# ToniChopp/ECAMP

Measured on AMD Instinct MI355X. Metric: pretrain image-report pairs/sec (ViT-B/16, 224^2, seq=128), higher is better.
Workload: dtype bf16

## Files before the change

### ecamp_amd/csrc/gemm.hip

```cpp
#include "common.h"
#include <stdlib.h>
#include <string.h>
#include <stdint.h>

#include "gemm_args.h"
void attn_set_head_mode(int on);
#include "gemm_q8.h"
#include "gemm_q16.h"

#define BM 128
#define BN 128
#define BK 64

__device__ __forceinline__ int swz(int row) { return (row >> 1) & 7; }

__device__ __forceinline__ void g2r_kc(const bf16_t* P, long ld, int row0, int nrows, int k0, int kend, int tid,
                                       uint4 (&r)[4]) {
#pragma unroll
    for (int i = 0; i < 4; ++i) {
        int c = tid + 256 * i;
        int row = c >> 3, kc = c & 7;
        int gr = row0 + row, gk = k0 + kc * 8;
        r[i] = (gr < nrows && gk < kend) ? *reinterpret_cast<const uint4*>(P + (long)gr * ld + gk) : make_uint4(0, 0, 0, 0);
    }
// ... 562 lines not shown
        }
    }
    hipLaunchKernelGGL(gemm_fp8_kernel, dim3(g.nbm * g.nbn), dim3(256), 0, stream, g, scale_a, scale_b);
    if (prof) ecamp_prof_end(stream);
    if (q8_out) {
        const long n4 = M * N / 4;
        int nb = (int)((n4 + 255) / 256);
        if (nb > 4096) nb = 4096;
        hipLaunchKernelGGL(quant_fp8_delayed_kernel<bf16_t>, dim3(nb), dim3(256), 0, stream, (const bf16_t*)C, q8_scale, (unsigned int*)q8_out, q8_amax_slots, n4);
    }
    ECAMP_LAUNCH_CHECK();
    return 0;
}

static int p8_num_cu() {
    static int ncu = 0;
    if (!ncu) {
        int dev = 0;
        (void)hipGetDevice(&dev);
        if (hipDeviceGetAttribute(&ncu, hipDeviceAttributeMultiprocessorCount, dev) != hipSuccess || ncu <= 0) ncu = 256;
        const char* cap = getenv("ECAMP_GEMM_GRID_CAP");
        if (cap && atoi(cap) >= 32 && atoi(cap) < ncu) {
            ncu = atoi(cap);
            fprintf(stderr, "[ecamp_hip] WARNING: ECAMP_GEMM_GRID_CAP=%d -- a development switch: every persistent GEMM of this process runs on %d "
                            "workgroups instead of one per CU\n", ncu, ncu);
        }
    }
    return ncu;
}
static int g_p8_wgrad = 1;
static int g_p8_wgrad_reserve = 0;
static int g_q8_bwd_grid = 0;

static int g_q8_mode = -2;
static int q8_env() {
    static const int v = getenv("ECAMP_GEMM_Q8") ? atoi(getenv("ECAMP_GEMM_Q8")) : -1;
    return g_q8_mode != -2 ? g_q8_mode : v;
}
static int q8_epi(const float* bias, const void* residual, const void* pre_out, const void* gmul, int act, int out_f32) {
    if (out_f32) return (!bias && !residual && !pre_out && !gmul && !act) ? 4 : -1;
    if (gmul) return (!bias && !pre_out && (act == 0 || act == 2)) ? 3 : -1;
    if (pre_out || act) return (pre_out && (act == 1 || act == 2) && !residual) ? 1 : -1;
    if (residual) return 2;
    return 0;
}
static long g_q8_launches = 0;
extern "C" int64_t ecamp_gemm_q8_launches(void) { return g_q8_launches; }
typedef void (*q8_fn)(GemmArgs);
static int g_q8_sch = -1;
static int q8_sch() {
    static const int v = getenv("ECAMP_Q8_SCH") ? atoi(getenv("ECAMP_Q8_SCH")) : 7;
    return g_q8_sch >= 0 ? g_q8_sch : v;
}
static q8_fn q8_pick(int a_kc, int b_kc, int epi, bool rowsum) {
    const int sch = q8_sch();
#define Q8S(A, B, E, R) ((q8_fn)gemm_bf16_q8_kernel<A, B, E, 0, R, 1>)
    if (a_kc && b_kc && (sch & 1)) return epi == 0 ? Q8S(true, true, 0, false) : epi == 1 ? Q8S(true, true, 1, false) : epi == 2 ? Q8S(true, true, 2, false) : (q8_fn) nullptr;
    if (a_kc && !b_kc && (sch & 2)) return epi == 0 ? Q8S(true, false, 0, false) : epi == 2 ? Q8S(true, false, 2, false) : epi == 3 ? Q8S(true, false, 3, false) : (q8_fn) nullptr;
    if (!a_kc && !b_kc && epi == 4 && (sch & 4)) return rowsum ? Q8S(false, false, 4, true) : Q8S(false, false, 4, false);
#undef Q8S
    if (a_kc && b_kc) return epi == 0 ? gemm_bf16_q8_kernel<true, true, 0> : epi == 1 ? gemm_bf16_q8_kernel<true, true, 1> : epi == 2 ? gemm_bf16_q8_kernel<true, true, 2> : (q8_fn) nullptr;
    if (a_kc && !b_kc) return epi == 0 ? gemm_bf16_q8_kernel<true, false, 0> : epi == 2 ? gemm_bf16_q8_kernel<true, false, 2> : epi == 3 ? gemm_bf16_q8_kernel<true, false, 3> : (q8_fn) nullptr;
    if (!a_kc && !b_kc && epi == 4) return rowsum ? gemm_bf16_q8_kernel<false, false, 4, 0, true> : gemm_bf16_q8_kernel<false, false, 4, 0, false>;
    return nullptr;
}
static bool q8_legal(const void* A, const void* B, const void* C, int64_t M, int64_t N, int64_t K, int a_kc, int64_t lda, int b_kc, int64_t ldb, int64_t ldc,
                     const float* bias, const void* residual, int64_t ldr, const void* pre_out, int64_t ldp, const void* gmul, int64_t ldg, int act,
                     int dtype, int out_f32, int split_k, const float* splitk_ws, const float* rowsum) {
    if (dtype != ECAMP_BF16) return false;
    const int epi = q8_epi(bias, residual, pre_out, gmul, act, out_f32);
    if (epi < 0 || !q8_pick(a_kc, b_kc, epi, rowsum != nullptr)) return false;
    if (split_k < 1) split_k = 1;
    if (split_k > 1 && epi != 4) return false;
    long kps = (K + split_k - 1) / split_k;
    kps = (kps + 63) / 64 * 64;
    const long ns = (K + kps - 1) / kps, last = K - (ns - 1) * kps;
    if (kps < 128 || last <= 64) return false;
    auto al16 = [](const void* q) { return (reinterpret_cast<uintptr_t>(q) & 15) == 0; };
    const long lim = 0x7fffffffl;
    if (N % 8 || lda % 8 || ldb % 8 || !al16(A) || !al16(B) || !al16(C)) return false;
    if ((a_kc ? M * lda : K * lda) * 2 > lim || (b_kc ? N * ldb : K * ldb) * 2 > lim) return false;
    if (!a_kc && M % 8) return false;
    if (split_k > 1) { if (!al16(splitk_ws) || (long)split_k * M * N * 4 > lim) return false; }
    else if (ldc % 8 || M * ldc * (epi == 4 ? 4 : 2) > lim) return false;
    if (bias && !al16(bias)) return false;
    if (pre_out && (ldp % 8 || !al16(pre_out) || M * ldp * 2 > lim)) return false;
    if (gmul && (ldg % 8 || !al16(gmul) || M * ldg * 2 > lim)) return false;
    if (residual && (ldr % 8 || !al16(residual) || M * ldr * 2 > lim)) return false;
    return true;
}

static int g_q16_mode = -1;
static int q16_mode() {
    static const int v = getenv("ECAMP_Q16") ? atoi(getenv("ECAMP_Q16")) : 1;
    return g_q16_mode >= 0 ? g_q16_mode : v;
}
static long g_q16_launches = 0;
extern "C" int64_t ecamp_gemm_q16_launches(void) { return g_q16_launches; }
static double q16_cost(int64_t M, int64_t N, int tn, int ncu) {
    const long tiles = (long)ceil_div(M, 256) * ceil_div(N, tn);
    return (double)((tiles + ncu - 1) / ncu) * (tn == 192 ? 0.79 : 1.0);
}
typedef void (*q16_fn)(GemmArgs);
static q16_fn q16_pick(int b_kc, int epi, int nw) {
    if (b_kc) {
        if (nw == 8) return epi == 0 ? (q16_fn)gemm_bf16_q16_kernel<0, 8, true> : (q16_fn)gemm_bf16_q16_kernel<2, 8, true>;
        return epi == 0 ? (q16_fn)gemm_bf16_q16_kernel<0, 6, true> : (q16_fn)gemm_bf16_q16_kernel<2, 6, true>;
    }
    if (nw == 8) return epi == 0 ? (q16_fn)gemm_bf16_q16_kernel<0, 8, false> : (q16_fn)gemm_bf16_q16_kernel<2, 8, false>;
    return epi == 0 ? (q16_fn)gemm_bf16_q16_kernel<0, 6, false> : (q16_fn)gemm_bf16_q16_kernel<2, 6, false>;
}

extern "C" int ecamp_set_option(const char* name, int32_t value) {
    ECAMP_CHECK_ARG(name != nullptr, "set_option: null name");
    if (strcmp(name, "q16_mode") == 0) { g_q16_mode = (value >= 0 && value <= 3) ? value : -1; return 0; }
    if (strcmp(name, "q8_mode") == 0) { g_q8_mode = (value == 0 || value == 2) ? value : -1; return 0; }
    if (strcmp(name, "p8_wgrad") == 0) { g_p8_wgrad = value ? 1 : 0; return 0; }
    if (strcmp(name, "p8_wgrad_reserve_cus") == 0) { g_p8_wgrad_reserve = value < 0 ? 0 : value; return 0; }
    if (strcmp(name, "q8_bwd_grid") == 0) { g_q8_bwd_grid = value < 0 ? 0 : value; return 0; }
    if (strcmp(name, "q8_sch") == 0) { g_q8_sch = value; return 0; }
    if (strcmp(name, "attn_head") == 0) { attn_set_head_mode(value); return 0; }
    return ecamp_set_error(-1, "set_option: unknown option '%s'", name);
}

static long q8_min_items() {
    static const long v = getenv("ECAMP_Q8_MIN_ITEMS") ? atol(getenv("ECAMP_Q8_MIN_ITEMS")) : (long)(0.5 * p8_num_cu());
    return v;
}
static long wgrad_target_items(int ncu) {
    static const long v = getenv("ECAMP_WGRAD_ITEMS") ? atol(getenv("ECAMP_WGRAD_ITEMS")) : 0;
    return v > 0 ? v : ncu;
}

extern "C" int ecamp_gemm_suggest_split(int64_t M, int64_t N, int64_t K, int a_kc, int b_kc, int dtype) {
    if (M <= 0 || N <= 0 || K <= 0) return 1;
    int ncu = p8_num_cu();
    if (!(a_kc && b_kc) && g_p8_wgrad_reserve > 0 && ncu - g_p8_wgrad_reserve >= 64) ncu -= g_p8_wgrad_reserve;
    const long tiles = (long)ceil_div(M, 128) * ceil_div(N, 128);
    long s_old = 1024 / tiles;
    if (s_old < 1) s_old = 1;
    const long cap = (K + 255) / 256;
    if (s_old > cap) s_old = cap;
    if (dtype != ECAMP_BF16 || q8_env() == 0 || (a_kc != 0) != (b_kc != 0) || (!a_kc && !b_kc && !g_p8_wgrad)) return (int)s_old;
    const long t8 = (long)ceil_div(M, 256) * ceil_div(N, 256);
    const long tgt = (!a_kc && !b_kc) ? wgrad_target_items(ncu) : ncu;
    int best = 1;
    double best_score = -1.0;
    for (int sp = 1; sp <= 32; ++sp) {
        if (sp > 1 && K / sp < 512) break;
        const long items = t8 * sp;
        const long rounds = (items + tgt - 1) / tgt;
        const double score = (double)items / (double)(rounds * tgt) - 0.012 * (sp - 1);
        if (score > best_score + 1e-9) { best_score = score; best = sp; }
    }
    return t8 * best >= q8_min_items() ? best : (int)s_old;
}

extern "C" int64_t ecamp_gemm_workspace_bytes(int64_t M, int64_t N, int64_t K, int32_t split_k) {
    (void)K;
    return split_k > 1 && M > 0 && N > 0 ? (int64_t)split_k * M * N * 4 : 0;
}

extern "C" int ecamp_gemm(const void* A, const void* B, void* C, int64_t M, int64_t N, int64_t K, int a_kc, int64_t lda,
                          int b_kc, int64_t ldb, int64_t ldc, const float* bias, const void* residual, int64_t ldr,
                          void* pre_out, int64_t ldp, const void* gmul, int64_t ldg, int act, float alpha, const float* alpha_dev, int dtype,
                          int out_f32, int accumulate, int split_k, float* splitk_ws, float* rowsum, hipStream_t stream) {
    ECAMP_CHECK_ARG(A && B && C, "ecamp_gemm: null operand");
    ECAMP_CHECK_ARG(M > 0 && N > 0 && K > 0, "ecamp_gemm: bad shape %ld %ld %ld", (long)M, (long)N, (long)K);
    ECAMP_CHECK_ARG(dtype == ECAMP_F32 || dtype == ECAMP_BF16, "ecamp_gemm: bad dtype %d", dtype);
    ECAMP_CHECK_ARG(act >= 0 && act <= 2, "ecamp_gemm: act=%d (0 none, 1 GELU, 2 GELU with the saved derivative)", act);
    ECAMP_CHECK_ARG(act != 2 || (dtype == ECAMP_BF16 && !out_f32 && ((pre_out != nullptr) != (gmul != nullptr))),
                    "ecamp_gemm: act=2 (saved derivative) is the bf16 forward form with pre_out or the data-gradient form with gmul");
    const int vec = dtype == ECAMP_BF16 ? 8 : 4;
// ... 390 lines not shown
```

### ecamp_amd/csrc/gemm_q8.h

```cpp
#pragma once
#include "gemm_args.h"
#include <type_traits>

typedef __attribute__((ext_vector_type(16))) float f32x16;
typedef hw_h16x8 hw_bf16x8;
typedef __attribute__((ext_vector_type(4))) short q8_v4s16;
typedef unsigned int q8_u32x4_t __attribute__((ext_vector_type(4)));

#define Q8_HALF 16384
#define Q8_GLDS16(SRC, DST) \
    __builtin_amdgcn_global_load_lds((const void __attribute__((address_space(1)))*)(SRC), (void __attribute__((address_space(3)))*)(DST), 16, 0, 0)

static __device__ __attribute__((aligned(16))) unsigned int q8_zero16[4] = {0u, 0u, 0u, 0u};

struct Q8Item {
    int m0, n0, kbeg, kend, nt, z, ncol;
};
template <int KT_SHIFT = 6>
__device__ __forceinline__ Q8Item q8_decode(const GemmArgs& g, int v, int total) {
    const unsigned f = (unsigned)xcd_remap(v, total), ntile = (unsigned)(g.nbm * g.nbn);
    const unsigned z = f / ntile, tile = f - z * ntile;
    const unsigned gw = 8u * (unsigned)g.nbn, grp = tile / gw, in = tile - grp * gw, first = grp * 8u;
    const unsigned gsz = min(8u, (unsigned)g.nbm - first);
    const unsigned nb = in / gsz, mb = first + (in - nb * gsz);
// ... 327 lines not shown
        } else {                                                                                                         \
            acc[tm_][nh_] = ECAMP_MFMA_32x32x16(FN[nh_].get(), FM[tm_].get(), (ZERO) ? zero16 : acc[tm_][nh_]); \
        }                                                                                                                \
    } while (0)

    const int esz = EPI == 4 ? 4 : 2;
    const long ldo = (EPI == 4 && g.partial) ? (long)g.N : g.ldc;
    const __amdgpu_buffer_rsrc_t rC = __builtin_amdgcn_make_buffer_rsrc(
        (EPI == 4 && g.partial) ? (void*)g.partial : g.C, 0,
        (int)(unsigned)(((EPI == 4 && g.partial) ? (long)g.nsplit * g.M : (long)g.M) * ldo * esz), 0x00020000);
    const __amdgpu_buffer_rsrc_t rP = __builtin_amdgcn_make_buffer_rsrc(EPI == 1 ? g.pre_out : g.C, 0, (int)(unsigned)((long)g.M * g.ldp * 2), 0x00020000);
    const __amdgpu_buffer_rsrc_t rQ = __builtin_amdgcn_make_buffer_rsrc((F8 && EPI == 1 && g.q8_out) ? g.q8_out : g.C, 0, (int)(unsigned)((long)g.M * g.ldc), 0x00020000);
    float q8_max = 0.f;
    const unsigned lane_o = (unsigned)((l31 * ldo + 8 * lh) * esz);
    const unsigned lane_p = (unsigned)((l31 * g.ldp + 8 * lh) * 2);
    const unsigned lane_g = (unsigned)((l31 * g.ldg + 8 * lh) * 2);
    const unsigned lane_r = (unsigned)((l31 * g.ldr + 8 * lh) * 2);
    const __amdgpu_buffer_rsrc_t rG = __builtin_amdgcn_make_buffer_rsrc((void*)(EPI == 3 ? g.gmul : g.C), 0, (int)(unsigned)((long)g.M * g.ldg * 2), 0x00020000);
    const __amdgpu_buffer_rsrc_t rR = __builtin_amdgcn_make_buffer_rsrc((void*)((EPI == 2 || EPI == 3) && g.residual ? g.residual : g.C), 0,
                                                                        (int)(unsigned)((long)g.M * g.ldr * 2), 0x00020000);
    q8_u32x4 bq[2][2][2];
    typedef unsigned q8_u32x4s __attribute__((ext_vector_type(4)));
    constexpr bool HAS_BIAS = (EPI <= 2) && !ITEMS;
    const unsigned bias_lane = (unsigned)((wc * 64 + 8 * lh) * 4);
    auto bias_request = [&](int tn0) __attribute__((always_inline)) {
        if constexpr (HAS_BIAS) {
            if (g.bias) {
                const unsigned long long bp = (unsigned long long)g.bias;
                const q8_u32x4s rs_ = {(unsigned)bp, (unsigned)(bp >> 32) & 0xffffu, (unsigned)g.N * 4u, 0x00020000u};
                const unsigned vo = (unsigned)tn0 * 4u + bias_lane;
#define Q8_BOF(NH_, GQ_, H_) "n"(((NH_) * 32 + (GQ_) * 16 + (H_) * 4) * 4)
                asm volatile("s_nop 4\n\t"
                             "buffer_load_dwordx4 %0, %8, %9, 0 offen offset:%10\n\t"
                             "buffer_load_dwordx4 %1, %8, %9, 0 offen offset:%11\n\t"
                             "buffer_load_dwordx4 %2, %8, %9, 0 offen offset:%12\n\t"
                             "buffer_load_dwordx4 %3, %8, %9, 0 offen offset:%13\n\t"
                             "buffer_load_dwordx4 %4, %8, %9, 0 offen offset:%14\n\t"
                             "buffer_load_dwordx4 %5, %8, %9, 0 offen offset:%15\n\t"
                             "buffer_load_dwordx4 %6, %8, %9, 0 offen offset:%16\n\t"
                             "buffer_load_dwordx4 %7, %8, %9, 0 offen offset:%17"
                             : "=&v"(bq[0][0][0]), "=&v"(bq[0][0][1]), "=&v"(bq[0][1][0]), "=&v"(bq[0][1][1]),
                               "=&v"(bq[1][0][0]), "=&v"(bq[1][0][1]), "=&v"(bq[1][1][0]), "=&v"(bq[1][1][1])
                             : "v"(vo), "s"(rs_), Q8_BOF(0, 0, 0), Q8_BOF(0, 0, 1), Q8_BOF(0, 1, 0), Q8_BOF(0, 1, 1),
                               Q8_BOF(1, 0, 0), Q8_BOF(1, 0, 1), Q8_BOF(1, 1, 0), Q8_BOF(1, 1, 1));
#undef Q8_BOF
            }
        }
    };
    auto bias_landed = [&]() __attribute__((always_inline)) {
        if constexpr (HAS_BIAS)
            asm volatile("" : "+v"(bq[0][0][0]), "+v"(bq[0][0][1]), "+v"(bq[0][1][0]), "+v"(bq[0][1][1]),
                              "+v"(bq[1][0][0]), "+v"(bq[1][0][1]), "+v"(bq[1][1][0]), "+v"(bq[1][1][1]));
    };
    auto store_quadrant = [&](int tm0, int tn0, int tz, auto mh_c, auto nh_c) {
        constexpr int MH = decltype(mh_c)::value, NH = decltype(nh_c)::value;
        constexpr int NTM = 2;
        if (DBG & 4) {
#pragma unroll
            for (int tm = 0; tm < NTM; ++tm) asm volatile("" ::"v"(acc[2 * MH + tm][NH]));
            return;
        }
        if constexpr (ITEMS) {
            const __amdgpu_buffer_rsrc_t rI = __builtin_amdgcn_make_buffer_rsrc((void*)uniform_ptr(gr_slabs + (long)tz * 65536), 0, 262144, 0x00020000);
#pragma unroll
            for (int tm = 0; tm < 2; ++tm)
#pragma unroll
                for (int gq = 0; gq < 2; ++gq) {
                    const unsigned o = (unsigned)((((wr * 128 + MH * 64 + tm * 32 + l31) * 256) + wc * 64 + NH * 32 + 16 * gq + 8 * lh) * 4);
                    const f32x16& a_ = acc[2 * MH + tm][NH];
                    __builtin_amdgcn_raw_buffer_store_b128((q8_u32x4){__float_as_uint(a_[8 * gq]), __float_as_uint(a_[8 * gq + 1]), __float_as_uint(a_[8 * gq + 2]), __float_as_uint(a_[8 * gq + 3])}, rI, o, 0, 0);
                    __builtin_amdgcn_raw_buffer_store_b128((q8_u32x4){__float_as_uint(a_[8 * gq + 4]), __float_as_uint(a_[8 * gq + 5]), __float_as_uint(a_[8 * gq + 6]), __float_as_uint(a_[8 * gq + 7])}, rI, o + 16, 0, 0);
                }
            return;
        }
        const int mb = tm0 + wr * 128 + MH * 64;
        const int nb = tn0 + wc * 64 + NH * 32;
        const bool edge = nb + 32 > g.N;
        typedef const float __attribute__((address_space(4))) cfloat4;
        float al = g.alpha;
        if (g.alpha_dev) {
            float ad = *(cfloat4*)g.alpha_dev;
            asm volatile("" : "+s"(ad));
            al *= ad;
        }
        if (F8 && g.alpha_dev2) {
            float ad = *(cfloat4*)g.alpha_dev2;
            asm volatile("" : "+s"(ad));
            al *= ad;
        }
        float bias[2][8];
#pragma unroll
        for (int gq = 0; gq < 2; ++gq)
#pragma unroll
            for (int r = 0; r < 8; ++r) bias[gq][r] = HAS_BIAS ? __uint_as_float(bq[NH][gq][r >> 2][r & 3]) : 0.f;
        unsigned uo[2][2], up[2][2], ug[2][2], ur[2][2];
#pragma unroll
        for (int tm = 0; tm < NTM; ++tm)
#pragma unroll
            for (int gq = 0; gq < 2; ++gq) {
                const long row = mb + tm * 32, col = nb + 16 * gq;
                const bool oob = (DBG & 1024) || (edge && (nb + 16 * gq + 8 * lh >= g.N)) || (EPI == 4 && g.partial && mb + tm * 32 + l31 >= g.M);
                uo[tm][gq] = oob ? 0x80000000u : (unsigned)(((EPI == 4 && g.partial ? (long)tz * g.M : 0) + row) * ldo + col) * esz + lane_o;
                if (EPI == 1) up[tm][gq] = oob ? 0x80000000u : (unsigned)((row * g.ldp + col) * 2) + lane_p;
                if (EPI == 3) ug[tm][gq] = oob ? 0x80000000u : (unsigned)((row * g.ldg + col) * 2) + lane_g;
                if (EPI == 2 || EPI == 3) ur[tm][gq] = oob ? 0x80000000u : (unsigned)((row * g.ldr + col) * 2) + lane_r;
            }
        float q8_inv = 0.f;
        if (F8 && EPI == 1 && g.q8_out) {
            float qs = *(cfloat4*)g.q8_scale;
            asm volatile("" : "+s"(qs));
            q8_inv = 1.0f / fmaxf(qs, 1e-30f);
        }
        q8_u32x4 qg[2][2], qr[2][2], qo[2][2][2];
#pragma unroll
        for (int tm = 0; tm < NTM; ++tm)
#pragma unroll
            for (int gq = 0; gq < 2; ++gq) {
                if (EPI == 3) qg[tm][gq] = __builtin_amdgcn_raw_buffer_load_b128(rG, ug[tm][gq], 0, 0);
                if (EPI == 2 || (EPI == 3 && g.residual)) qr[tm][gq] = __builtin_amdgcn_raw_buffer_load_b128(rR, ur[tm][gq], 0, 0);
                if (EPI == 4 && !g.partial && g.accumulate) {
                    qo[tm][gq][0] = __builtin_amdgcn_raw_buffer_load_b128(rC, uo[tm][gq], 0, 0);
                    qo[tm][gq][1] = __builtin_amdgcn_raw_buffer_load_b128(rC, uo[tm][gq] + 16, 0, 0);
                }
            }
#pragma unroll
        for (int tm = 0; tm < NTM; ++tm)
#pragma unroll
            for (int gq = 0; gq < 2; ++gq) {
                float v[8];
#pragma unroll
                for (int r = 0; r < 8; ++r) v[r] = acc[2 * MH + tm][NH][8 * gq + r] * al;
                if (EPI <= 2 && g.bias) {
#pragma unroll
                    for (int r = 0; r < 8; ++r) v[r] += bias[gq][r];
                }
                if (EPI == 1) {
                    if (g.act == 2) {
                        float d_[8];
#pragma unroll
                        for (int r = 0; r < 8; r += 2) {
                            f32x2_t g_;
                            const f32x2_t y_ = gelu_both_fast_f2((f32x2_t){rnd<bf16_t>(v[r]), rnd<bf16_t>(v[r + 1])}, g_);
                            v[r] = y_[0]; v[r + 1] = y_[1];
                            d_[r] = g_[0]; d_[r + 1] = g_[1];
                        }
                        __builtin_amdgcn_raw_buffer_store_b128(q8_pack8(d_), rP, up[tm][gq], 0, ST_AUX);
                    } else {
                    __builtin_amdgcn_raw_buffer_store_b128(q8_pack8(v), rP, up[tm][gq], 0, ST_AUX);
#pragma unroll
                    for (int r = 0; r < 8; r += 2) {
                        const f32x2_t y_ = gelu_fast_f2((f32x2_t){rnd<bf16_t>(v[r]), rnd<bf16_t>(v[r + 1])});
                        v[r] = y_[0]; v[r + 1] = y_[1];
                    }
                    }
                    if (F8 && g.q8_out) {
                        float u[8];
                        const bool row_in = mb + tm * 32 + l31 < g.M && uo[tm][gq] != 0x80000000u;
#pragma unroll
                        for (int r = 0; r < 8; ++r) {
                            const float yr = rnd<bf16_t>(v[r]);
                            if (row_in) q8_max = fmaxf(q8_max, fabsf(yr));
                            u[r] = fminf(fmaxf(yr * q8_inv, -448.f), 448.f);
                        }
                        int w0 = 0, w1 = 0;
                        w0 = __builtin_amdgcn_cvt_pk_fp8_f32(u[0], u[1], w0, false); w0 = __builtin_amdgcn_cvt_pk_fp8_f32(u[2], u[3], w0, true);
                        w1 = __builtin_amdgcn_cvt_pk_fp8_f32(u[4], u[5], w1, false); w1 = __builtin_amdgcn_cvt_pk_fp8_f32(u[6], u[7], w1, true);
                        typedef unsigned int q8_u32x2_ __attribute__((ext_vector_type(2)));
                        __builtin_amdgcn_raw_buffer_store_b64((q8_u32x2_){(unsigned)w0, (unsigned)w1}, rQ, uo[tm][gq] == 0x80000000u ? 0x80000000u : (uo[tm][gq] >> 1), 0, 0);
                    }
                }
                if (EPI == 3) {
#pragma unroll
                    for (int r = 0; r < 4; ++r) {
                        const f32x2_t lg_ = {h16_lo(qg[tm][gq][r]), h16_hi(qg[tm][gq][r])};
                        const f32x2_t gp_ = g.act == 2 ? lg_ : gelu_grad_fast_f2(lg_);
                        v[2 * r] *= gp_[0];
                        v[2 * r + 1] *= gp_[1];
                    }
                }
                if (EPI == 2 || (EPI == 3 && g.residual)) {
#pragma unroll
                    for (int r = 0; r < 4; ++r) {
                        v[2 * r] += h16_lo(qr[tm][gq][r]);
                        v[2 * r + 1] += h16_hi(qr[tm][gq][r]);
                    }
                }
                if (EPI == 4) {
                    if (!g.partial && g.accumulate) {
#pragma unroll
                        for (int r = 0; r < 4; ++r) { v[r] += __uint_as_float(qo[tm][gq][0][r]); v[4 + r] += __uint_as_float(qo[tm][gq][1][r]); }
                    }
                    __builtin_amdgcn_raw_buffer_store_b128((q8_u32x4){__float_as_uint(v[0]), __float_as_uint(v[1]), __float_as_uint(v[2]), __float_as_uint(v[3])}, rC, uo[tm][gq], 0, 0);
                    __builtin_amdgcn_raw_buffer_store_b128((q8_u32x4){__float_as_uint(v[4]), __float_as_uint(v[5]), __float_as_uint(v[6]), __float_as_uint(v[7])}, rC, uo[tm][gq] + 16, 0, 0);
                } else {
                    __builtin_amdgcn_raw_buffer_store_b128(q8_pack8(v), rC, uo[tm][gq], 0, ST_AUX);
                }
            }
    };
    const __amdgpu_buffer_rsrc_t rS = __builtin_amdgcn_make_buffer_rsrc((void*)(ROWSUM && g.rowsum ? (void*)g.rowsum : g.C), 0, (int)(unsigned)((long)g.M * 4), 0x00020000);
    auto rowsum_flush = [&]() {
        typedef const float __attribute__((address_space(4))) cfloat4;
        float al = ITEMS ? Q8_PROB(rsp_prob, alpha_out) : g.alpha_out;
        const float* adp = ITEMS ? (const float*)uniform_ptr(Q8_PROB(rsp_prob, alpha_dev_out)) : g.alpha_dev_out;
        if (adp) { float ad = *(cfloat4*)adp; asm volatile("" : "+s"(ad)); al *= ad; }
        __amdgpu_buffer_rsrc_t rSi = rS;
        if (ITEMS) rSi = __builtin_amdgcn_make_buffer_rsrc((void*)uniform_ptr(Q8_PROB(rsp_prob, rowsum)), 0, (int)(unsigned)((long)Q8_PROB(rsp_prob, M) * 4), 0x00020000);
#pragma unroll
        for (int t = 0; t < 4; ++t) {
            const float tot = (rsp[t] + __shfl_xor(rsp[t], 32, 64)) * al;
            const unsigned off = lh ? 0x80000000u : (unsigned)((rsp_m0 + wr * 128 + t * 32 + l31) * 4);
            __builtin_amdgcn_raw_ptr_buffer_atomic_fadd_f32(tot, rSi, off, 0, 0);
        }
        rsp_on = false;
    };
    using I0 = std::integral_constant<int, 0>;
    using I1 = std::integral_constant<int, 1>;
    const f32x16 zero16 = {0.f, 0.f, 0.f, 0.f, 0.f, 0.f, 0.f, 0.f, 0.f, 0.f, 0.f, 0.f, 0.f, 0.f, 0.f, 0.f};
#define Q8_STORE_Q(TM0, TN0, TZ, Q)                                                           \
    do {                                                                                      \
        if ((Q) == 0) store_quadrant(TM0, TN0, TZ, I0(), I0());                               \
        if ((Q) == 1) store_quadrant(TM0, TN0, TZ, I0(), I1());                               \
        if ((Q) == 2) store_quadrant(TM0, TN0, TZ, I1(), I1());                               \
        if ((Q) == 3) store_quadrant(TM0, TN0, TZ, I1(), I0());                               \
    } while (0)
#define Q8_SB() __builtin_amdgcn_sched_barrier(0)
#define Q8_PHASE(KS, DPART, WAIT, ZERO, PRE_HOOK)                                                                     \
    do {                                                                                                                 \
        if (PRE_HOOK) {                                                                                                  \
            if (have_pend) { Q8_STORE_Q(pm0, pn0, pz, 0); Q8_STORE_Q(pm0, pn0, pz, 1); Q8_STORE_Q(pm0, pn0, pz, 2); Q8_STORE_Q(pm0, pn0, pz, 3); } \
            bias_request(cn0);                                                                                           \
            if (ROWSUM) { if (rsp_on) rowsum_flush(); }                                                                  \
            Q8_SB();                                                                                                     \
        }                                                                                                                \
        Q8_READ_GROUP(xm, xn, sM, sN, KS); Q8_SB();                                                                      \
        Q8_STAGE_PART(DPART); Q8_SB();                                                                                   \
        if (WAIT) { if (pdone) Q8_WAIT_DMA(0); else Q8_WAIT_DMA(4); }      \
        if (!A_KC || !B_KC) { q8_wait4(xm); q8_wait2(xn); }                                                              \
        asm volatile("s_waitcnt lgkmcnt(0)" ::: "memory"); Q8_SB();                                                      \
        if (!(DBG & 16)) __builtin_amdgcn_s_barrier();                                                                   \
        Q8_SB();                                                                                                         \
        if (!(DBG & 8)) __builtin_amdgcn_s_setprio(1);                                                                   \
        if (ROWSUM) { Q8_RS_ACC(xm); }             \
        Q8_MFMA1(xm, xn, 0, ZERO); Q8_MFMA1(xm, xn, 1, ZERO); Q8_MFMA1(xm, xn, 2, ZERO); Q8_MFMA1(xm, xn, 3, ZERO);      \
        Q8_MFMA1(xm, xn, 4, ZERO); Q8_MFMA1(xm, xn, 5, ZERO); Q8_MFMA1(xm, xn, 6, ZERO); Q8_MFMA1(xm, xn, 7, ZERO);      \
        Q8_SB();                                                                                                         \
        if (!(DBG & 8)) __builtin_amdgcn_s_setprio(0);                                                                   \
        if (!(DBG & 16)) __builtin_amdgcn_s_barrier();                                                                   \
        Q8_SB();                                                                                                         \
    } while (0)
#define Q8_KTILE(FIRST)                                                                                               \
    do {                                                                                                                 \
        const int ra_ = rA + wr, rb_ = rB + (wc >> 1);                                                                   \
        const unsigned char* sM = lds + (ra_ >= NSLOT ? ra_ - NSLOT : ra_) * Q8_HALF;                                    \
        const unsigned char* sN = lds + (NSLOT + (rb_ >= NSLOT ? rb_ - NSLOT : rb_)) * Q8_HALF;                          \
        Q8_PHASE(0, 2, false, FIRST, FIRST);                                                                          \
        Q8_PHASE(1, 3, false, false, false);                                                                          \
        Q8_PHASE(2, 0, false, false, false);                                                                          \
        Q8_PHASE(3, 1, true, false, false);                                                                           \
        rA = rA + 2 >= NSLOT ? rA + 2 - NSLOT : rA + 2;                                                                  \
        rB = rB + 2 >= NSLOT ? rB + 2 - NSLOT : rB + 2;                                                                  \
    } while (0)

#define Q9_PHASE(KS, DPART, WAIT, ZERO, PRE_HOOK, MX_HOOK)                                                              \
    do {                                                                                                                 \
        if (PRE_HOOK) {                                                                                                  \
            if (have_pend) { Q8_STORE_Q(pm0, pn0, pz, 0); Q8_STORE_Q(pm0, pn0, pz, 1); Q8_STORE_Q(pm0, pn0, pz, 2); Q8_STORE_Q(pm0, pn0, pz, 3); } \
            bias_request(cn0);                                                                                           \
            if (ROWSUM) { if (rsp_on) rowsum_flush(); }                                                                  \
            Q8_SB();                                                                                                     \
        }                                                                                                                \
        Q8_READ_GROUP(xm, xn, sM, sN, KS); Q8_SB();                                                                      \
        Q9_ISSUE(DPART); Q8_SB();                                                                                        \
        Q9_ADVANCE(DPART); Q8_SB();                                                                                      \
        if (WAIT) Q8_WAIT_DMA(4);                                                                                        \
        if (!A_KC || !B_KC) { q8_wait4(xm); q8_wait2(xn); }                                                              \
        asm volatile("s_waitcnt lgkmcnt(0)" ::: "memory"); Q8_SB();                                                      \
        if (!(DBG & 16)) __builtin_amdgcn_s_barrier();                                                                   \
        Q8_SB();                                                                                                         \
        if (!(DBG & 8)) __builtin_amdgcn_s_setprio(1);                                                                   \
        Q8_MFMA1(xm, xn, 0, ZERO); Q8_MFMA1(xm, xn, 1, ZERO); Q8_SB();                                                   \
        Q8_MFMA1(xm, xn, 2, ZERO); Q8_MFMA1(xm, xn, 3, ZERO); Q8_SB();                                                   \
        if (MX_HOOK) { if (cv + G < total) Q9_CDECODE(cv + G); }                                                           \
        Q8_SB();                                                                                                         \
        if (ROWSUM) { Q8_RS_ACC(xm); }    \
        Q8_MFMA1(xm, xn, 4, ZERO); Q8_MFMA1(xm, xn, 5, ZERO); Q8_MFMA1(xm, xn, 6, ZERO); Q8_MFMA1(xm, xn, 7, ZERO);      \
        Q8_SB();                                                                                                         \
        if (!(DBG & 8)) __builtin_amdgcn_s_setprio(0);                                                                   \
        if (!(DBG & 16)) __builtin_amdgcn_s_barrier();                                                                   \
        Q8_SB();                                                                                                         \
    } while (0)
    Q8Frag8 ym[2], yn[2];
#define Q9F_MFMA(TMI, NH, ZERO)                                                                                          \
    acc[2 * MH_ + (TMI)][NH] = __builtin_amdgcn_mfma_scale_f32_32x32x64_f8f6f4(yn[NH].get(), ym[TMI].get(), (ZERO) ? zero16 : acc[2 * MH_ + (TMI)][NH], \
                                                                               0, 0, 0, 0x7F7F7F7F, 0, 0x7F7F7F7F)
#define Q9F_PHASE(KS8, MH, DPART, WAIT, ZERO, PRE_HOOK, MX_HOOK)                                                         \
    do {                                                                                                                 \
        constexpr int MH_ = (MH);                                                                                        \
        if (PRE_HOOK) {                                                                                                  \
            if (have_pend) { Q8_STORE_Q(pm0, pn0, pz, 0); Q8_STORE_Q(pm0, pn0, pz, 1); Q8_STORE_Q(pm0, pn0, pz, 2); Q8_STORE_Q(pm0, pn0, pz, 3); } \
            bias_request(cn0);                                                                                           \
            Q8_SB();                                                                                                     \
        }                                                                                                                \
        if ((MH) == 0) {                                                                                                 \
            yn[0].template read<0>(sN + offN[2 * (KS8)], sN + offN[2 * (KS8) + 1]);                                       \
        }                                                                                                                \
        ym[0].template read<(2 * (MH)) * 4096>(sM + offM[2 * (KS8)], sM + offM[2 * (KS8) + 1]);                           \
        ym[1].template read<(2 * (MH) + 1) * 4096>(sM + offM[2 * (KS8)], sM + offM[2 * (KS8) + 1]);                       \
        if ((MH) == 0) {                                                                                                 \
            yn[1].template read<4096>(sN + offN[2 * (KS8)], sN + offN[2 * (KS8) + 1]);                                    \
        }                                                                                                                \
        Q8_SB();                                                                                                         \
        Q9_ISSUE(DPART); Q8_SB();                                                                                        \
        if (WAIT) Q8_WAIT_DMA(4);                                                                                        \
        asm volatile("s_waitcnt lgkmcnt(0)" ::: "memory"); Q8_SB();                                                      \
        __builtin_amdgcn_s_barrier();                                                                                    \
        Q8_SB();                                                                                                         \
        __builtin_amdgcn_s_setprio(1);                                                                                   \
        Q9F_MFMA(0, 0, ZERO); Q9F_MFMA(0, 1, ZERO); Q8_SB();                                                             \
        Q9_ADVANCE(DPART);                      \
        if (MX_HOOK) { if (cv + G < total) Q9_CDECODE(cv + G); }                                                         \
        Q8_SB();                                                                                                         \
        Q9F_MFMA(1, 1, ZERO); Q9F_MFMA(1, 0, ZERO);                                                                      \
        Q8_SB();                                                                                                         \
        __builtin_amdgcn_s_setprio(0);                                                                                   \
        __builtin_amdgcn_s_barrier();                                                                                    \
        Q8_SB();                                                                                                         \
    } while (0)
#define Q9F_KTILE(FIRST)                                                                                              \
    do {                                                                                                                 \
        const int ra_ = rA + wr, rb_ = rB + (wc >> 1);                                                                   \
        const unsigned char* sM = lds + (ra_ >= NSLOT ? ra_ - NSLOT : ra_) * Q8_HALF;                                    \
        const unsigned char* sN = lds + (NSLOT + (rb_ >= NSLOT ? rb_ - NSLOT : rb_)) * Q8_HALF;                          \
        Q9F_PHASE(0, 0, 2, false, FIRST, FIRST, false);                                                               \
        Q9F_PHASE(0, 1, 3, false, FIRST, false, FIRST);                                                               \
        Q9F_PHASE(1, 0, 0, false, false, false, false);                                                               \
        Q9F_PHASE(1, 1, 1, true, false, false, false);                                                                \
        rA = rA + 2 >= NSLOT ? rA + 2 - NSLOT : rA + 2;                                                                  \
        rB = rB + 2 >= NSLOT ? rB + 2 - NSLOT : rB + 2;                                                                  \
    } while (0)
#define Q9_KTILE(FIRST)                                                                                               \
    do {                                                                                                                 \
        const int ra_ = rA + wr, rb_ = rB + (wc >> 1);                                                                   \
        const unsigned char* sM = lds + (ra_ >= NSLOT ? ra_ - NSLOT : ra_) * Q8_HALF;                                    \
        const unsigned char* sN = lds + (NSLOT + (rb_ >= NSLOT ? rb_ - NSLOT : rb_)) * Q8_HALF;                          \
        Q9_PHASE(0, 2, false, FIRST, FIRST, false);                                                                   \
        Q9_PHASE(1, 3, false, false, false, FIRST);                                                                   \
        Q9_PHASE(2, 0, false, false, false, false);                                                                   \
        Q9_PHASE(3, 1, true, false, false, false);                                                                    \
        rA = rA + 2 >= NSLOT ? rA + 2 - NSLOT : rA + 2;                                                                  \
        rB = rB + 2 >= NSLOT ? rB + 2 - NSLOT : rB + 2;                                                                  \
    } while (0)

// ... 32 lines not shown
            nm0 = cr.m0; nn0 = cr.prob; nz = cr.slab; ncnt = (cr.kend - cr.kbeg + 63) >> 6;                              \
            if (ROWSUM) nrs = (cr.flags & 1) != 0 && wc == 0 && Q8_PROB(cr.prob, rowsum) != nullptr;                     \
        } else {                                                                                                         \
            const Q8Item cit = q8_decode<KT_SHIFT>(g, V_, total);                                                        \
            nm0 = cit.m0; nn0 = cit.n0; nz = cit.z; ncnt = cit.nt;                                                       \
            if (ROWSUM) nrs = g.rowsum != nullptr && wc == 0 && cit.ncol == 0;                                           \
        }                                                                                                                \
    } while (0)
    if constexpr (SCH != 0) {
        if (it_beg < total) Q9_CDECODE(it_beg);
        for (int cv = it_beg; cv < total; cv += G) {
            const int cm0 = nm0, cn0 = nn0, cz = nz, cnt = ncnt;
            if (ROWSUM) { rs_on = nrs; rs_ones = rs_on ? H16_ONE_X2 : 0u; }
            if constexpr (F8) {
                Q9F_KTILE(true); bias_landed();
#pragma unroll 1
                for (int t = 1; t < cnt; ++t) Q9F_KTILE(false);
            } else {
                Q9_KTILE(true); bias_landed();
#pragma unroll 1
                for (int t = 1; t < cnt; ++t) Q9_KTILE(false);
            }
            have_pend = true; pm0 = cm0; pn0 = cn0; pz = cz;
            if (ROWSUM) {
                rsp_on = rs_on; rsp_m0 = cm0; rsp_prob = cn0;
#pragma unroll
                for (int t = 0; t < 4; ++t) { rsp[t] = rs[t]; rs[t] = 0.f; }
            }
        }
        Q8_WAIT_DMA(0);
    } else
    for (int cv = it_beg; cv < total; cv += G) {
        int cm0, cn0, cz, cnt;
        if (ITEMS) {
            const Q8ItemRec cr = item_at(cv);
            cm0 = cr.m0; cn0 = cr.prob; cz = cr.slab; cnt = (cr.kend - cr.kbeg + 63) >> 6;
            if (ROWSUM) { rs_on = (cr.flags & 1) != 0 && wc == 0 && Q8_PROB(cr.prob, rowsum) != nullptr; rs_ones = rs_on ? H16_ONE_X2 : 0u; }
        } else {
            const Q8Item cit = q8_decode(g, cv, total);
            cm0 = cit.m0; cn0 = cit.n0; cz = cit.z; cnt = cit.nt;
            if (ROWSUM) { rs_on = g.rowsum != nullptr && wc == 0 && cit.ncol == 0; rs_ones = rs_on ? H16_ONE_X2 : 0u; }
        }
        Q8_KTILE(true); bias_landed();
#pragma unroll 1
        for (int t = 1; t < cnt; ++t) Q8_KTILE(false);
        have_pend = true; pm0 = cm0; pn0 = cn0; pz = cz;
        if (ROWSUM) {
            rsp_on = rs_on; rsp_m0 = cm0; rsp_prob = cn0;
#pragma unroll
            for (int t = 0; t < 4; ++t) { rsp[t] = rs[t]; rs[t] = 0.f; }
        }
    }
    if (wr == 0) __builtin_amdgcn_s_barrier();
    if (have_pend) { Q8_STORE_Q(pm0, pn0, pz, 0); Q8_STORE_Q(pm0, pn0, pz, 1); Q8_STORE_Q(pm0, pn0, pz, 2); Q8_STORE_Q(pm0, pn0, pz, 3); }
    if (ROWSUM) { if (rsp_on) rowsum_flush(); }
    if (F8 && EPI == 1 && g.q8_out) {
#pragma unroll
        for (int o = 32; o > 0; o >>= 1) q8_max = fmaxf(q8_max, __shfl_xor(q8_max, o, 64));
        if (lane == 0) atomicMax(reinterpret_cast<unsigned int*>(g.q8_amax + ((blockIdx.x + wave) & 15) * 32), __float_as_uint(q8_max));
    }
#undef Q8_STORE_Q
#undef Q8_SB
#undef Q8_READ_GROUP
#undef Q8_MFMA1
#undef Q8_RD1
#undef Q8_STAGE_PART
#undef Q8_STAGE_PCS
#undef Q8_RS_ACC
#undef Q8_KTILE
#undef Q8_PHASE
#undef Q9_KTILE
#undef Q9F_KTILE
#undef Q9F_PHASE
#undef Q9F_MFMA
#undef Q9_PHASE
#undef Q9_ISSUE
#undef Q9_ADVANCE
#undef Q9_ITEM
#undef Q9_CDECODE
#undef Q8_NEXT_ITEM
#undef Q8_WAIT_DMA
}
#undef Q8_PROB
#undef Q8_VAL_

template <bool A_KC, bool B_KC, int EPI, int DBG = 0, bool ROWSUM = false, int SCH = 0>
__global__ __launch_bounds__(512) void gemm_bf16_q8_kernel(GemmArgs g) {
    Q8Group none;
    q8_body<A_KC, B_KC, EPI, DBG, ROWSUM, false, SCH>(g, none);
}
template <int EPI>
__global__ __launch_bounds__(512) void gemm_f8_q8_kernel(GemmArgs g) {
    Q8Group none;
    q8_body<true, true, EPI, 0, false, false, 1, true>(g, none);
}
template <bool ROWSUM, int SCH = 0>
__global__ __launch_bounds__(512) void gemm_bf16_q8_items_kernel(GemmArgs g, Q8Group GR) {
    q8_body<false, false, 4, 0, ROWSUM, true, SCH>(g, GR);
}
```

Baseline: 7367.

## Transpose GEMM epilogue in registers to store full contiguous row lines

```diff
diff --git a/ecamp_amd/csrc/gemm.hip b/ecamp_amd/csrc/gemm.hip
--- a/ecamp_amd/csrc/gemm.hip
+++ b/ecamp_amd/csrc/gemm.hip
@@ -638,12 +638,20 @@
     static const int v = getenv("ECAMP_Q8_SCH") ? atoi(getenv("ECAMP_Q8_SCH")) : 7;
     return g_q8_sch >= 0 ? g_q8_sch : v;
 }
+static int g_q8_epi = -1;
+static int q8_epi_lines() {
+    static const int v = getenv("ECAMP_Q8_EPI") ? atoi(getenv("ECAMP_Q8_EPI")) : 1;
+    return g_q8_epi >= 0 ? g_q8_epi : v;
+}
 static q8_fn q8_pick(int a_kc, int b_kc, int epi, bool rowsum) {
-    const int sch = q8_sch();
+    const int sch = q8_sch(), lm = q8_epi_lines();
+    const bool lines = lm >= 2 || (lm == 1 && (epi == 0 || epi == 2));
 #define Q8S(A, B, E, R) ((q8_fn)gemm_bf16_q8_kernel<A, B, E, 0, R, 1>)
-    if (a_kc && b_kc && (sch & 1)) return epi == 0 ? Q8S(true, true, 0, false) : epi == 1 ? Q8S(true, true, 1, false) : epi == 2 ? Q8S(true, true, 2, false) : (q8_fn) nullptr;
-    if (a_kc && !b_kc && (sch & 2)) return epi == 0 ? Q8S(true, false, 0, false) : epi == 2 ? Q8S(true, false, 2, false) : epi == 3 ? Q8S(true, false, 3, false) : (q8_fn) nullptr;
+#define Q8L(A, B, E) (lines ? (q8_fn)gemm_bf16_q8_kernel<A, B, E, 0, false, 1> : (q8_fn)gemm_bf16_q8_kernel<A, B, E, 2048, false, 1>)
+    if (a_kc && b_kc && (sch & 1)) return epi == 0 ? Q8L(true, true, 0) : epi == 1 ? Q8L(true, true, 1) : epi == 2 ? Q8L(true, true, 2) : (q8_fn) nullptr;
+    if (a_kc && !b_kc && (sch & 2)) return epi == 0 ? Q8L(true, false, 0) : epi == 2 ? Q8L(true, false, 2) : epi == 3 ? Q8L(true, false, 3) : (q8_fn) nullptr;
     if (!a_kc && !b_kc && epi == 4 && (sch & 4)) return rowsum ? Q8S(false, false, 4, true) : Q8S(false, false, 4, false);
+#undef Q8L
 #undef Q8S
     if (a_kc && b_kc) return epi == 0 ? gemm_bf16_q8_kernel<true, true, 0> : epi == 1 ? gemm_bf16_q8_kernel<true, true, 1> : epi == 2 ? gemm_bf16_q8_kernel<true, true, 2> : (q8_fn) nullptr;
     if (a_kc && !b_kc) return epi == 0 ? gemm_bf16_q8_kernel<true, false, 0> : epi == 2 ? gemm_bf16_q8_kernel<true, false, 2> : epi == 3 ? gemm_bf16_q8_kernel<true, false, 3> : (q8_fn) nullptr;
@@ -705,6 +713,7 @@
     if (strcmp(name, "p8_wgrad_reserve_cus") == 0) { g_p8_wgrad_reserve = value < 0 ? 0 : value; return 0; }
     if (strcmp(name, "q8_bwd_grid") == 0) { g_q8_bwd_grid = value < 0 ? 0 : value; return 0; }
     if (strcmp(name, "q8_sch") == 0) { g_q8_sch = value; return 0; }
+    if (strcmp(name, "q8_epi") == 0) { g_q8_epi = value; return 0; }
     if (strcmp(name, "attn_head") == 0) { attn_set_head_mode(value); return 0; }
     return ecamp_set_error(-1, "set_option: unknown option '%s'", name);
 }
diff --git a/ecamp_amd/csrc/gemm_q8.h b/ecamp_amd/csrc/gemm_q8.h
--- a/ecamp_amd/csrc/gemm_q8.h
+++ b/ecamp_amd/csrc/gemm_q8.h
@@ -403,6 +403,61 @@
             asm volatile("" : "+v"(bq[0][0][0]), "+v"(bq[0][0][1]), "+v"(bq[0][1][0]), "+v"(bq[0][1][1]),
                               "+v"(bq[1][0][0]), "+v"(bq[1][0][1]), "+v"(bq[1][1][0]), "+v"(bq[1][1][1]));
     };
+    auto epi_alpha = [&]() __attribute__((always_inline)) {
+        typedef const float __attribute__((address_space(4))) cfloat4;
+        float al = g.alpha;
+        if (g.alpha_dev) {
+            float ad = *(cfloat4*)g.alpha_dev;
+            asm volatile("" : "+s"(ad));
+            al *= ad;
+        }
+        if (F8 && g.alpha_dev2) {
+            float ad = *(cfloat4*)g.alpha_dev2;
+            asm volatile("" : "+s"(ad));
+            al *= ad;
+        }
+        return al;
+    };
+    auto epi_math = [&](float (&v)[8], float (&p)[8], const float (&bias8)[8], q8_u32x4 qg, q8_u32x4 qr) __attribute__((always_inline)) {
+        if (EPI <= 2 && g.bias) {
+#pragma unroll
+            for (int r = 0; r < 8; ++r) v[r] += bias8[r];
+        }
+        if (EPI == 1) {
+            if (g.act == 2) {
+#pragma unroll
+                for (int r = 0; r < 8; r += 2) {
+                    f32x2_t g_;
+                    const f32x2_t y_ = gelu_both_fast_f2((f32x2_t){rnd<bf16_t>(v[r]), rnd<bf16_t>(v[r + 1])}, g_);
+                    v[r] = y_[0]; v[r + 1] = y_[1];
+                    p[r] = g_[0]; p[r + 1] = g_[1];
+                }
+            } else {
+#pragma unroll
+                for (int r = 0; r < 8; r += 2) {
+                    p[r] = v[r]; p[r + 1] = v[r + 1];
+                    const f32x2_t y_ = gelu_fast_f2((f32x2_t){rnd<bf16_t>(v[r]), rnd<bf16_t>(v[r + 1])});
+                    v[r] = y_[0]; v[r + 1] = y_[1];
+                }
+            }
+        }
+        if (EPI == 3) {
+#pragma unroll
+            for (int r = 0; r < 4; ++r) {
+                const f32x2_t lg_ = {h16_lo(qg[r]), h16_hi(qg[r])};
+                const f32x2_t gp_ = g.act == 2 ? lg_ : gelu_grad_fast_f2(lg_);
+                v[2 * r] *= gp_[0];
+                v[2 * r + 1] *= gp_[1];
+            }
+        }
+        if (EPI == 2 || (EPI == 3 && g.residual)) {
+#pragma unroll
+            for (int r = 0; r < 4; ++r) {
+                v[2 * r] += h16_lo(qr[r]);
+                v[2 * r + 1] += h16_hi(qr[r]);
+            }
+        }
+    };
     auto store_quadrant = [&](int tm0, int tn0, int tz, auto mh_c, auto nh_c) {
         constexpr int MH = decltype(mh_c)::value, NH = decltype(nh_c)::value;
         constexpr int NTM = 2;
@@ -428,17 +483,7 @@
         const int nb = tn0 + wc * 64 + NH * 32;
         const bool edge = nb + 32 > g.N;
         typedef const float __attribute__((address_space(4))) cfloat4;
-        float al = g.alpha;
-        if (g.alpha_dev) {
-            float ad = *(cfloat4*)g.alpha_dev;
-            asm volatile("" : "+s"(ad));
-            al *= ad;
-        }
-        if (F8 && g.alpha_dev2) {
-            float ad = *(cfloat4*)g.alpha_dev2;
-            asm volatile("" : "+s"(ad));
-            al *= ad;
-        }
+        const float al = epi_alpha();
         float bias[2][8];
 #pragma unroll
         for (int gq = 0; gq < 2; ++gq)
@@ -478,32 +523,12 @@
         for (int tm = 0; tm < NTM; ++tm)
 #pragma unroll
             for (int gq = 0; gq < 2; ++gq) {
-                float v[8];
+                float v[8], p[8];
 #pragma unroll
                 for (int r = 0; r < 8; ++r) v[r] = acc[2 * MH + tm][NH][8 * gq + r] * al;
-                if (EPI <= 2 && g.bias) {
-#pragma unroll
-                    for (int r = 0; r < 8; ++r) v[r] += bias[gq][r];
-                }
+                if (EPI <= 3) epi_math(v, p, bias[gq], qg[tm][gq], qr[tm][gq]);
                 if (EPI == 1) {
-                    if (g.act == 2) {
-                        float d_[8];
-#pragma unroll
-                        for (int r = 0; r < 8; r += 2) {
-                            f32x2_t g_;
-                            const f32x2_t y_ = gelu_both_fast_f2((f32x2_t){rnd<bf16_t>(v[r]), rnd<bf16_t>(v[r + 1])}, g_);
-                            v[r] = y_[0]; v[r + 1] = y_[1];
-                            d_[r] = g_[0]; d_[r + 1] = g_[1];
-                        }
-                        __builtin_amdgcn_raw_buffer_store_b128(q8_pack8(d_), rP, up[tm][gq], 0, ST_AUX);
-                    } else {
-                    __builtin_amdgcn_raw_buffer_store_b128(q8_pack8(v), rP, up[tm][gq], 0, ST_AUX);
-#pragma unroll
-                    for (int r = 0; r < 8; r += 2) {
-                        const f32x2_t y_ = gelu_fast_f2((f32x2_t){rnd<bf16_t>(v[r]), rnd<bf16_t>(v[r + 1])});
-                        v[r] = y_[0]; v[r + 1] = y_[1];
-                    }
-                    }
+                    __builtin_amdgcn_raw_buffer_store_b128(q8_pack8(p), rP, up[tm][gq], 0, ST_AUX);
                     if (F8 && g.q8_out) {
                         float u[8];
                         const bool row_in = mb + tm * 32 + l31 < g.M && uo[tm][gq] != 0x80000000u;
@@ -520,22 +545,6 @@
                         __builtin_amdgcn_raw_buffer_store_b64((q8_u32x2_){(unsigned)w0, (unsigned)w1}, rQ, uo[tm][gq] == 0x80000000u ? 0x80000000u : (uo[tm][gq] >> 1), 0, 0);
                     }
                 }
-                if (EPI == 3) {
-#pragma unroll
-                    for (int r = 0; r < 4; ++r) {
-                        const f32x2_t lg_ = {h16_lo(qg[tm][gq][r]), h16_hi(qg[tm][gq][r])};
-                        const f32x2_t gp_ = g.act == 2 ? lg_ : gelu_grad_fast_f2(lg_);
-                        v[2 * r] *= gp_[0];
-                        v[2 * r + 1] *= gp_[1];
-                    }
-                }
-                if (EPI == 2 || (EPI == 3 && g.residual)) {
-#pragma unroll
-                    for (int r = 0; r < 4; ++r) {
-                        v[2 * r] += h16_lo(qr[tm][gq][r]);
-                        v[2 * r + 1] += h16_hi(qr[tm][gq][r]);
-                    }
-                }
                 if (EPI == 4) {
                     if (!g.partial && g.accumulate) {
 #pragma unroll
@@ -548,6 +557,75 @@
                 }
             }
     };
+    const bool x_b3 = (lane >> 3) & 1;
+    auto xpose = [&](q8_u32x4 (&x)[4]) __attribute__((always_inline)) {
+#pragma unroll
+        for (int d = 0; d < 4; ++d) {
+#pragma unroll
+            for (int k = 0; k < 2; ++k) {
+                const auto s_ = __builtin_amdgcn_permlane16_swap(x[k][d], x[k + 2][d], false, false);
+                x[k][d] = s_[0]; x[k + 2][d] = s_[1];
+            }
+#pragma unroll
+            for (int k = 0; k < 4; k += 2) {
+                const unsigned a_ = x[k][d], b_ = x[k + 1][d];
+                const unsigned pa_ = (unsigned)__builtin_amdgcn_update_dpp(0, (int)a_, 0x128, 0xf, 0xf, false);
+                const unsigned pb_ = (unsigned)__builtin_amdgcn_update_dpp(0, (int)b_, 0x128, 0xf, 0xf, false);
+                x[k][d] = x_b3 ? pb_ : a_;
+                x[k + 1][d] = x_b3 ? b_ : pa_;
+            }
+        }
+    };
+    const int x_col = 32 * ((lane >> 4) & 1) + 16 * x_b3 + 8 * lh, x_row = lane & 7;
+    auto store_half = [&](int tm0, int tn0, auto mh_c) {
+        constexpr int MH = decltype(mh_c)::value;
+        if (DBG & 4) {
+#pragma unroll
+            for (int tm = 0; tm < 2; ++tm) asm volatile("" ::"v"(acc[2 * MH + tm][0]), "v"(acc[2 * MH + tm][1]));
+            return;
+        }
+        const int mb = tm0 + wr * 128 + MH * 64;
+        const int col = tn0 + wc * 64 + x_col;
+        const bool oob = (DBG & 1024) || col >= g.N;
+        const float al = epi_alpha();
+        auto off = [&](long ld, int tm, int s) __attribute__((always_inline)) {
+            return oob ? 0x80000000u : (unsigned)(((long)(mb + tm * 32 + x_row + 8 * (s & 1) + 16 * (s >> 1)) * ld + col) * 2);
+        };
+#pragma unroll
+        for (int tm = 0; tm < 2; ++tm) {
+            q8_u32x4 qg[4], qr[4];
+#pragma unroll
+            for (int s = 0; s < 4; ++s) {
+                if (EPI == 3) qg[s] = __builtin_amdgcn_raw_buffer_load_b128(rG, off(g.ldg, tm, s), 0, 0);
+                if (EPI == 2 || (EPI == 3 && g.residual)) qr[s] = __builtin_amdgcn_raw_buffer_load_b128(rR, off(g.ldr, tm, s), 0, 0);
+            }
+            if (EPI == 3) xpose(qg);
+            if (EPI == 2 || (EPI == 3 && g.residual)) xpose(qr);
+            q8_u32x4 xc[4], xp[4];
+#pragma unroll
+            for (int nh = 0; nh < 2; ++nh)
+#pragma unroll
+                for (int gq = 0; gq < 2; ++gq) {
+                    float bias8[8], v[8], p[8];
+#pragma unroll
+                    for (int r = 0; r < 8; ++r) {
+                        bias8[r] = HAS_BIAS ? __uint_as_float(bq[nh][gq][r >> 2][r & 3]) : 0.f;
+                        v[r] = acc[2 * MH + tm][nh][8 * gq + r] * al;
+                    }
+                    epi_math(v, p, bias8, qg[2 * nh + gq], qr[2 * nh + gq]);
+                    xc[2 * nh + gq] = q8_pack8(v);
+                    if (EPI == 1) xp[2 * nh + gq] = q8_pack8(p);
+                }
+            xpose(xc);
+            if (EPI == 1) xpose(xp);
+#pragma unroll
+            for (int s = 0; s < 4; ++s) {
+                if (EPI == 1) __builtin_amdgcn_raw_buffer_store_b128(xp[s], rP, off(g.ldp, tm, s), 0, ST_AUX);
+                __builtin_amdgcn_raw_buffer_store_b128(xc[s], rC, off(ldo, tm, s), 0, ST_AUX);
+            }
+        }
+    };
+    constexpr bool LINES = !F8 && !ITEMS && EPI <= 3 && !(DBG & 2048);
     const __amdgpu_buffer_rsrc_t rS = __builtin_amdgcn_make_buffer_rsrc((void*)(ROWSUM && g.rowsum ? (void*)g.rowsum : g.C), 0, (int)(unsigned)((long)g.M * 4), 0x00020000);
     auto rowsum_flush = [&]() {
         typedef const float __attribute__((address_space(4))) cfloat4;
@@ -574,11 +652,16 @@
         if ((Q) == 2) store_quadrant(TM0, TN0, TZ, I1(), I1());                               \
         if ((Q) == 3) store_quadrant(TM0, TN0, TZ, I1(), I0());                               \
     } while (0)
+#define Q8_STORE_TILE(TM0, TN0, TZ)                                                                                      \
+    do {                                                                                                                 \
+        if constexpr (LINES) { store_half(TM0, TN0, I0()); store_half(TM0, TN0, I1()); }                                 \
+        else { Q8_STORE_Q(TM0, TN0, TZ, 0); Q8_STORE_Q(TM0, TN0, TZ, 1); Q8_STORE_Q(TM0, TN0, TZ, 2); Q8_STORE_Q(TM0, TN0, TZ, 3); } \
+    } while (0)
 #define Q8_SB() __builtin_amdgcn_sched_barrier(0)
 #define Q8_PHASE(KS, DPART, WAIT, ZERO, PRE_HOOK)                                                                     \
     do {                                                                                                                 \
         if (PRE_HOOK) {                                                                                                  \
-            if (have_pend) { Q8_STORE_Q(pm0, pn0, pz, 0); Q8_STORE_Q(pm0, pn0, pz, 1); Q8_STORE_Q(pm0, pn0, pz, 2); Q8_STORE_Q(pm0, pn0, pz, 3); } \
+            if (have_pend) Q8_STORE_TILE(pm0, pn0, pz); \
             bias_request(cn0);                                                                                           \
             if (ROWSUM) { if (rsp_on) rowsum_flush(); }                                                                  \
             Q8_SB();                                                                                                     \
@@ -615,7 +698,7 @@
 #define Q9_PHASE(KS, DPART, WAIT, ZERO, PRE_HOOK, MX_HOOK)                                                              \
     do {                                                                                                                 \
         if (PRE_HOOK) {                                                                                                  \
-            if (have_pend) { Q8_STORE_Q(pm0, pn0, pz, 0); Q8_STORE_Q(pm0, pn0, pz, 1); Q8_STORE_Q(pm0, pn0, pz, 2); Q8_STORE_Q(pm0, pn0, pz, 3); } \
+            if (have_pend) Q8_STORE_TILE(pm0, pn0, pz); \
             bias_request(cn0);                                                                                           \
             if (ROWSUM) { if (rsp_on) rowsum_flush(); }                                                                  \
             Q8_SB();                                                                                                     \
@@ -648,7 +731,7 @@
     do {                                                                                                                 \
         constexpr int MH_ = (MH);                                                                                        \
         if (PRE_HOOK) {                                                                                                  \
-            if (have_pend) { Q8_STORE_Q(pm0, pn0, pz, 0); Q8_STORE_Q(pm0, pn0, pz, 1); Q8_STORE_Q(pm0, pn0, pz, 2); Q8_STORE_Q(pm0, pn0, pz, 3); } \
+            if (have_pend) Q8_STORE_TILE(pm0, pn0, pz); \
             bias_request(cn0);                                                                                           \
             Q8_SB();                                                                                                     \
         }                                                                                                                \
@@ -787,7 +870,7 @@
         }
     }
     if (wr == 0) __builtin_amdgcn_s_barrier();
-    if (have_pend) { Q8_STORE_Q(pm0, pn0, pz, 0); Q8_STORE_Q(pm0, pn0, pz, 1); Q8_STORE_Q(pm0, pn0, pz, 2); Q8_STORE_Q(pm0, pn0, pz, 3); }
+    if (have_pend) Q8_STORE_TILE(pm0, pn0, pz);
     if (ROWSUM) { if (rsp_on) rowsum_flush(); }
     if (F8 && EPI == 1 && g.q8_out) {
 #pragma unroll
@@ -795,6 +878,7 @@
         if (lane == 0) atomicMax(reinterpret_cast<unsigned int*>(g.q8_amax + ((blockIdx.x + wave) & 15) * 32), __float_as_uint(q8_max));
     }
 #undef Q8_STORE_Q
+#undef Q8_STORE_TILE
 #undef Q8_SB
 #undef Q8_READ_GROUP
 #undef Q8_MFMA1
```

Result: no change. 7362, median of 6 (-0.1%).
